# AIBluefisher/DAGSfM

Measured on AMD Instinct MI355X. Metric: verified image-pairs/sec (+ RANSAC hypotheses/sec) at 4096 feats/image, higher is better.
Workload: dtype u8 matching (int8 MFMA) + f64 verification

## Files before the change

dagsfm_amd/capi.py:

```python
import ctypes
import os

import numpy as np

_HERE = os.path.dirname(os.path.abspath(__file__))
LIB_PATH = os.environ.get("DSM_LIB_PATH") or os.path.join(_HERE, "libdagsfm_mi355x.so")
CHECK_LIB_PATH = os.environ.get("DSM_CHECK_LIB_PATH") or os.path.join(_HERE, "libdagsfm_mi355x_check.so")

GATHER_LIB_PATH = os.path.join(_HERE, "libdagsfm_gather.so")

u8p = ctypes.POINTER(ctypes.c_uint8)
u32p = ctypes.POINTER(ctypes.c_uint32)
u64p = ctypes.POINTER(ctypes.c_uint64)
f32p = ctypes.POINTER(ctypes.c_float)


class DsmError(RuntimeError):
    pass


class MatchOptions(ctypes.Structure):
    _fields_ = [("max_ratio", ctypes.c_double), ("max_distance", ctypes.c_double),
                ("cross_check", ctypes.c_int32), ("max_num_matches", ctypes.c_int32)]

# ... 668 lines not shown
            "image_camera": np.array([cam_new[int(icam[i])] for i in images], np.uint32),
            "qvec": qvec[images].copy(), "tvec": tvec[images].copy(), "image_constant_pose": cpose, "image_constant_tvec": cmask,
            "point_ids": ids[points].copy(), "xyz": xyz[points].copy(), "point_constant": np.array(pconst, np.uint8),
            "track_offsets": np.concatenate([[0], np.cumsum([len(t) for t in tracks])]).astype(np.uint32),
            "obs_image": np.array([img_new[int(oimg[k])] for t in tracks for k in t], np.uint32),
            "obs_xy": (np.concatenate([oxy[t] for t in tracks]) if tracks else np.zeros((0, 2))).reshape(-1, 2),
            "image_index": np.array(images, np.int64), "camera_index": np.array(cams, np.int64),
            "point_index": np.array(points, np.int64)}


def absolute_pose_seed(problem, factor_index, user_seed=0):
    return int(lib().dsm_absolute_pose_seed(problem, factor_index, user_seed))


def absolute_pose_factors(options=None):
    o = options if options is not None else default_absolute_pose_options()
    n = int(lib().dsm_absolute_pose_factors(ctypes.byref(o), None, 0))
    out = np.zeros(max(n, 1))
    lib().dsm_absolute_pose_factors(ctypes.byref(o), out.ctypes.data, n)
    return out[:n].copy()


def absolute_pose_max_trials(options=None):
    o = options if options is not None else default_absolute_pose_options()
    return int(lib().dsm_absolute_pose_max_trials(ctypes.byref(o)))


def align_seed(i, j, direction, user_seed=0):
    return int(lib().dsm_align_seed(i, j, direction, user_seed))


PRODUCT_OPTION_KEYS = ("DSM_MATCH_CHUNK_ROWS", "DSM_VERIFY_CHUNK_PAIRS", "DSM_VERIFY_LANES", "DSM_VERIFY_INLINE_LO", "DSM_VERIFY_ITEM_MODE",
                       "DSM_LO_TAIL", "DSM_LO_TAIL_MODE", "DSM_VERIFY_GRID_DIV")
CHECK_OPTION_KEYS = ("DSM_K1_DOT4", "DSM_VERIFY_DEBUG", "DSM_SAMPLER_SERIAL", "DSM_LO_PREPARE_WAVE", "DSM_LO_JACOBI_GROUPS", "DSM_ROOTS_LDS",
                     "DSM_FINAL_WAVES", "DSM_VERIFY_LEGACY", "DSM_VERIFY_FIXED_BATCH", "DSM_VERIFY_LANE_SPLIT", "DSM_DEBUG_SAMPLER_MODE",
                     "DSM_VOCAB_ASSIGN_VALU", "DSM_VERIFY_HOST_LOOP", "DSM_SCORE_PREFILTER", "DSM_VERIFY_REPLAY_GRID", "DSM_REPLAY_LEGACY", "DSM_FLANN_GROUP", "DSM_FLANN_STATS", "DSM_ELU_LDS", "DSM_HYP_GRID", "DSM_SPEC_MARGIN",
                     "DSM_POSE_FULL")
DEBUG_OPTION_KEYS = PRODUCT_OPTION_KEYS


def check_requested():
    return os.environ.get("DSM_LIBRARY") == "check" or any(os.environ.get(k) is not None for k in CHECK_OPTION_KEYS)


class Context:

    def __init__(self, device=0, check=None):
        self._handle = ctypes.c_void_p()
        self._debug = {}
        self.check = check_requested() if check is None else bool(check)
        self._L = lib(self.check)
        rc = self._L.dsm_ctx_create(device, ctypes.byref(self._handle))
        if rc != 0:
            raise DsmError("dsm_ctx_create failed (%d): %s" % (rc, self._L.dsm_last_error(None).decode()))
        self.n_pairs = 0

    @property
    def _h(self):
        if self._handle:
            for key in PRODUCT_OPTION_KEYS + CHECK_OPTION_KEYS:
                want = os.environ.get(key)
                if self._debug.get(key) != want:
                    self.set_debug_option(key, want)
        return self._handle

    def set_memory_budget(self, nbytes):
        self._L.dsm_ctx_set_memory_budget.argtypes = [ctypes.c_void_p, ctypes.c_uint64]
# ... 858 lines not shown
```

dagsfm_amd/csrc/capi.hip:

```cpp
#include <hip/hip_runtime.h>
#include <math.h>
#include <stdint.h>
#include <stdio.h>
#include <stdlib.h>
#include <string.h>

#include <algorithm>
#include <string>
#include <system_error>
#include <thread>
#include <vector>

#include "../../include/dagsfm_mi355x.h"
#include "ctx.h"
#include "kernels.h"
#include "verify_camera.h"

namespace {
thread_local std::string g_create_error;
}

static const uint64_t kStageSlot = 16ull << 20;
static const uint64_t kStageSmall = 1ull << 20;
static const unsigned kStageThreads = 8;
// ... 428 lines not shown
    uint32_t c1 = c0;
    while (c1 < n_pairs) {
      const uint64_t r = ctx->rows[pairs[2 * c1]];
      if (c1 > c0 && rows_acc + r > budget_rows) break;
      rows_acc += r;
      ++c1;
    }
    const uint32_t nc = c1 - c0;
    dpairs.resize(nc);
    dpairs2.resize(nc);
    pdir.resize(nc);
    doff.resize(nc);
    order.resize(nc);
    std::fill(cnt_b.begin(), cnt_b.end(), 0u);
    uint64_t off = 0;
    uint32_t max_rb = 0;
    for (uint32_t k = 0; k < nc; ++k) {
      const uint32_t a = pairs[2 * (c0 + k)], b = pairs[2 * (c0 + k) + 1];
      dpairs[k] = make_uint2(a, b);
      dpairs2[k] = make_uint2(b, a);
      pdir[k] = make_uint4(k, 0, ctx->nfeat[a], ctx->nfeat[b]);
      doff[k] = off;
      off += ctx->rows[a];
      max_rb = std::max(max_rb, ctx->rows[a] / 256);
      cnt_b[b + 1]++;
    }
    for (uint32_t k = 0; k < ctx->n_images; ++k) cnt_b[k + 1] += cnt_b[k];
    for (uint32_t k = 0; k < nc; ++k) order[cnt_b[dpairs[k].y]++] = k;
    HIPCHK(ctx, ctx->d_dpairs.reserve(std::max<uint32_t>(nc, 1) * sizeof(uint2)));
    HIPCHK(ctx, ctx->d_order.reserve(std::max<uint32_t>(nc, 1) * 4));
    HIPCHK(ctx, ctx->d_doutoff.reserve(std::max<uint32_t>(nc, 1) * 8));
    HIPCHK(ctx, ctx->d_pair_dir.reserve(std::max<uint32_t>(nc, 1) * sizeof(uint4)));
    HIPCHK(ctx, ctx->d_m.reserve(std::max<uint64_t>(off, 1) * 4));
    HIPCHK(ctx, ctx->d_ms.reserve(std::max<uint64_t>(off, 1) * 4));
    HIPCHK(ctx, hipMemcpyAsync(ctx->d_dpairs.p, dpairs.data(), nc * sizeof(uint2), hipMemcpyHostToDevice, st));
    HIPCHK(ctx, hipMemcpyAsync(ctx->d_order.p, order.data(), nc * 4, hipMemcpyHostToDevice, st));
    HIPCHK(ctx, hipMemcpyAsync(ctx->d_doutoff.p, doff.data(), nc * 8, hipMemcpyHostToDevice, st));
    HIPCHK(ctx, hipMemcpyAsync(ctx->d_pair_dir.p, pdir.data(), nc * sizeof(uint4), hipMemcpyHostToDevice, st));

    K1Params k1;
    k1.desc = ctx->d_desc.as<int8_t>();
    k1.rterm = ctx->d_rterm.as<int32_t>();
    k1.dpairs = ctx->d_dpairs.as<uint2>();
    k1.img_row0 = ctx->d_img_row0.as<uint32_t>();
    k1.img_rows = ctx->d_img_rows.as<uint32_t>();
    k1.d_out_off = ctx->d_doutoff.as<uint64_t>();
    k1.lut = ctx->d_lut.as<float>();
    k1.max_ratio = (float)options->max_ratio;
    k1.max_distance = (float)options->max_distance;
    k1.out = ctx->d_m.as<int32_t>();
    k1.out_s = ctx->d_ms.as<int32_t>();
    k1.order = ctx->d_order.as<uint32_t>();
    k1.entries = nullptr;
    k1.e_off = nullptr;
    k1.e_cnt = nullptr;
    while (ctx->ev.size() < ev_used + 6) {
      DevEvent e;
      HIPCHK(ctx, hipEventCreate(&e.e));
      ctx->ev.push_back(std::move(e));
    }
#ifdef DSM_CHECK_BUILD
    const bool k1_dot4 = ctx->dbg("DSM_K1_DOT4") != nullptr;
#else
    const bool k1_dot4 = false;
#endif
    HIPCHK(ctx, hipEventRecord(ctx->ev[ev_used], st));
#ifdef DSM_CHECK_BUILD
    if (k1_dot4)
      launch_k1_dot4(k1, nc, max_rb, st);
    else
#endif
      launch_k1(k1, nc, max_rb, st);
    HIPCHK(ctx, hipGetLastError());
    HIPCHK(ctx, hipEventRecord(ctx->ev[ev_used + 1], st));
    if (!k1_dot4) launch_k1_resolve(k1, nc, max_rb, st);
    HIPCHK(ctx, hipGetLastError());
    HIPCHK(ctx, hipEventRecord(ctx->ev[ev_used + 2], st));
    if (max_rb) ctx->k1_launches++;

    K2Params k2;
    k2.pair_dir = ctx->d_pair_dir.as<uint4>();
    k2.d_out_off = ctx->d_doutoff.as<uint64_t>();
    k2.m = ctx->d_m.as<int32_t>();
    k2.cross_check = 0;
    k2.matches = nullptr;
    uint64_t total = 0;
    if (!cross) {
      HIPCHK(ctx, hipEventRecord(ctx->ev[ev_used + 3], st));
      HIPCHK(ctx, hipEventRecord(ctx->ev[ev_used + 4], st));
      k2.counts = ctx->d_counts.as<uint32_t>() + c0;
      k2.offsets = ctx->d_offsets.as<uint64_t>() + c0;
      launch_k2(k2, nc, false, st);
      HIPCHK(ctx, hipGetLastError());
      launch_scan(ctx->d_counts.as<uint32_t>() + c0, ctx->d_offsets.as<uint64_t>() + c0, nc, ctx->d_total.as<uint64_t>(), st);
      HIPCHK(ctx, hipGetLastError());
      HIPCHK(ctx, hipMemcpyAsync(&total, ctx->d_total.p, 8, hipMemcpyDeviceToHost, st));
      HIPCHK(ctx, hipStreamSynchronize(st));
      HIPCHK(ctx, ctx->d_matches.grow(std::max<uint64_t>(total, 1) * 8, ctx->total_matches * 8, st));
      k2.matches = ctx->d_matches.as<uint32_t>();
      launch_k2(k2, nc, true, st);
      HIPCHK(ctx, hipGetLastError());
    } else {
      HIPCHK(ctx, ctx->d_ecnt.reserve(std::max<uint32_t>(nc, 1) * 4));
      HIPCHK(ctx, ctx->d_eoff.reserve(((size_t)nc + 1) * 8));
      HIPCHK(ctx, ctx->d_etotal.reserve(8));
      HIPCHK(ctx, hipMemsetAsync(ctx->d_etotal.p, 0, 8, st));
      k2.counts = ctx->d_ecnt.as<uint32_t>();
      k2.offsets = ctx->d_eoff.as<uint64_t>();
      launch_k2(k2, nc, false, st);
      HIPCHK(ctx, hipGetLastError());
      launch_scan(ctx->d_ecnt.as<uint32_t>(), ctx->d_eoff.as<uint64_t>(), nc, ctx->d_etotal.as<uint64_t>(), st);
      HIPCHK(ctx, hipGetLastError());
      uint64_t etotal = 0;
      HIPCHK(ctx, hipMemcpyAsync(&etotal, ctx->d_etotal.p, 8, hipMemcpyDeviceToHost, st));
      HIPCHK(ctx, hipStreamSynchronize(st));
      HIPCHK(ctx, ctx->d_entries.reserve(std::max<uint64_t>(etotal, 1) * 8));
      HIPCHK(ctx, ctx->d_out2.reserve(std::max<uint64_t>(etotal, 1) * 4));
      HIPCHK(ctx, ctx->d_out2s.reserve(std::max<uint64_t>(etotal, 1) * 4));
      k2.matches = ctx->d_entries.as<uint32_t>();
      launch_k2(k2, nc, true, st);
      HIPCHK(ctx, hipGetLastError());
      HIPCHK(ctx, ctx->d_dpairs2.reserve(std::max<uint32_t>(nc, 1) * sizeof(uint2)));
      HIPCHK(ctx, hipMemcpyAsync(ctx->d_dpairs2.p, dpairs2.data(), nc * sizeof(uint2), hipMemcpyHostToDevice, st));
      K1Params g = k1;
      g.dpairs = ctx->d_dpairs2.as<uint2>();
      g.order = nullptr;
      g.entries = ctx->d_entries.as<uint2>();
      g.e_off = ctx->d_eoff.as<uint64_t>();
      g.e_cnt = ctx->d_ecnt.as<uint32_t>();
      g.out = ctx->d_out2.as<int32_t>();
      g.out_s = ctx->d_out2s.as<int32_t>();
      HIPCHK(ctx, hipEventRecord(ctx->ev[ev_used + 3], st));
      if (etotal) {
        launch_k1(g, nc, max_rb, st);
        HIPCHK(ctx, hipGetLastError());
      }
      HIPCHK(ctx, hipEventRecord(ctx->ev[ev_used + 4], st));
      if (etotal) {
        launch_k1_resolve(g, nc, max_rb, st);
        HIPCHK(ctx, hipGetLastError());
      }
      K2eParams ke;
      ke.entries = g.entries;
      ke.e_off = g.e_off;
      ke.e_cnt = g.e_cnt;
      ke.out2 = ctx->d_out2.as<int32_t>();
      ke.counts = ctx->d_counts.as<uint32_t>() + c0;
      ke.offsets = ctx->d_offsets.as<uint64_t>() + c0;
      ke.matches = nullptr;
      launch_k2_entries(ke, nc, false, st);
      HIPCHK(ctx, hipGetLastError());
      launch_scan(ctx->d_counts.as<uint32_t>() + c0, ctx->d_offsets.as<uint64_t>() + c0, nc, ctx->d_total.as<uint64_t>(), st);
      HIPCHK(ctx, hipGetLastError());
      HIPCHK(ctx, hipMemcpyAsync(&total, ctx->d_total.p, 8, hipMemcpyDeviceToHost, st));
      HIPCHK(ctx, hipStreamSynchronize(st));
      HIPCHK(ctx, ctx->d_matches.grow(std::max<uint64_t>(total, 1) * 8, ctx->total_matches * 8, st));
      ke.matches = ctx->d_matches.as<uint32_t>();
      launch_k2_entries(ke, nc, true, st);
      HIPCHK(ctx, hipGetLastError());
    }
    HIPCHK(ctx, hipEventRecord(ctx->ev[ev_used + 5], st));
    ev_used += 6;
    ctx->total_matches = total;
    HIPCHK(ctx, hipStreamSynchronize(st));
    c0 = c1;
  }
  HIPCHK(ctx, hipStreamSynchronize(st));
  for (size_t k = 0; k + 5 < ev_used; k += 6) {
    float ms = 0.f;
    HIPCHK(ctx, hipEventElapsedTime(&ms, ctx->ev[k + 4], ctx->ev[k + 5]));
    ctx->k1t_ms += ms;
    HIPCHK(ctx, hipEventElapsedTime(&ms, ctx->ev[k + 2], ctx->ev[k + 3]));
    ctx->k1t_ms += ms;
    HIPCHK(ctx, hipEventElapsedTime(&ms, ctx->ev[k], ctx->ev[k + 1]));
// ... 1243 lines not shown
```

dagsfm_amd/csrc/ctx.h:

```cpp
#ifndef DAGSFM_AMD_CSRC_CTX_H_
#define DAGSFM_AMD_CSRC_CTX_H_

#include <hip/hip_runtime.h>
#include <stdint.h>

#include <map>
#include <string>
#include <vector>

#include "../../include/dagsfm_mi355x.h"

struct DevBuf {
  void* p = nullptr;
  size_t cap = 0;
  DevBuf() = default;
  DevBuf(const DevBuf&) = delete;
  DevBuf& operator=(const DevBuf&) = delete;
  DevBuf(DevBuf&& o) noexcept : p(o.p), cap(o.cap) {
    o.p = nullptr;
    o.cap = 0;
  }
  DevBuf& operator=(DevBuf&& o) noexcept {
    if (this != &o) {
      release();
// ... 167 lines not shown

  struct RetrievalState* retrieval = nullptr;
  struct CovSiftState* covsift = nullptr;
  struct SiftState* sift = nullptr;

  std::vector<double> cluster_ritz, cluster_vectors;
  uint32_t cluster_rows = 0, cluster_cols = 0;

  template <typename F>
  void for_each_buffer(F f) {
    for (DevBuf* b : {&d_desc, &d_rterm, &d_kp, &d_img_row0, &d_img_rows, &d_lut, &d_stage, &d_counts, &d_offsets, &d_matches, &d_total, &d_etotal,
                      &d_cams, &d_pairs_dev, &d_seeds, &d_tvg, &d_inl, &d_inl_counts, &d_inl_off, &d_inl_compact, &d_inl_total, &d_nt_table,
                      &d_nt_off, &d_nt_off_t, &d_pair_state, &d_pts_px, &d_pts_norm, &d_reports, &d_masks, &d_fam_state, &d_sidx, &d_lo_inl,
                      &d_nt_table_t, &d_wm_redo, &d_wm_total, &d_wm_count, &d_lo_inl_pool, &d_pose_jobs,
                      &d_g_nfeat, &d_g_dpairs, &d_g_doff, &d_g_pdir, &d_g_params, &d_g_m, &d_g_counts, &d_g_offsets, &d_g_total, &d_g_matches,
                      &d_g_plan, &d_g_inl, &d_g_inl_off,
                      &d_mm_matches[0], &d_mm_matches[1], &d_mm_off[0], &d_mm_off[1], &d_mm_counts, &d_mm_state, &d_mm_first, &d_mm_acc,
                      &d_mm_keep, &d_mm_total})
      f(*b, false);
    for (DevBuf* b : {&d_m, &d_ms, &d_entries, &d_out2, &d_out2s, &d_dpairs, &d_dpairs2, &d_doutoff, &d_pair_dir, &d_order, &d_ecnt, &d_eoff,
                      &d_vscratch})
      f(*b, true);
    for (VerifyLane& L : lanes) L.for_each_buffer([&f](DevBuf& b) { f(b, true); });
  }
};
void dsm_retrieval_destroy(dsm_ctx* ctx);
void dsm_retrieval_invalidate(dsm_ctx* ctx);
void dsm_sift_destroy(dsm_ctx* ctx);
void dsm_covariant_sift_destroy(dsm_ctx* ctx);

static const char* const dsm_product_debug_keys[] = {"DSM_MATCH_CHUNK_ROWS", "DSM_VERIFY_CHUNK_PAIRS", "DSM_VERIFY_LANES", "DSM_VERIFY_INLINE_LO",
                                                     "DSM_VERIFY_ITEM_MODE", "DSM_LO_TAIL", "DSM_LO_TAIL_MODE", "DSM_VERIFY_GRID_DIV"};
#ifdef DSM_CHECK_BUILD
static const char* const dsm_check_debug_keys[] = {"DSM_K1_DOT4", "DSM_VERIFY_DEBUG", "DSM_SAMPLER_SERIAL", "DSM_LO_PREPARE_WAVE", "DSM_LO_JACOBI_GROUPS",
                                                   "DSM_ROOTS_LDS", "DSM_FINAL_WAVES", "DSM_VERIFY_LEGACY", "DSM_VERIFY_FIXED_BATCH", "DSM_VERIFY_LANE_SPLIT",
                                                   "DSM_DEBUG_SAMPLER_MODE", "DSM_VOCAB_ASSIGN_VALU", "DSM_VERIFY_HOST_LOOP", "DSM_SCORE_PREFILTER",
                                                   "DSM_VERIFY_REPLAY_GRID", "DSM_REPLAY_LEGACY", "DSM_FLANN_GROUP", "DSM_FLANN_STATS", "DSM_ELU_LDS", "DSM_HYP_GRID", "DSM_SPEC_MARGIN",
                                                   "DSM_POSE_FULL"};
#endif

#define HIPCHK(ctx, call)                                                              \
  do {                                                                                 \
    hipError_t e_ = (call);                                                            \
    if (e_ != hipSuccess) {                                                            \
      (ctx)->err = std::string(#call) + ": " + hipGetErrorString(e_);                  \
      return DSM_ERR_HIP;                                                              \
    }                                                                                  \
  } while (0)

#define HIPTRY(call)                                                   \
  do {                                                                 \
    hipError_t e_ = (call);                                            \
    if (e_ != hipSuccess && rc == DSM_OK) {                            \
      ctx->err = std::string(#call) + ": " + hipGetErrorString(e_);    \
      rc = DSM_ERR_HIP;                                                \
    }                                                                  \
  } while (0)

static inline int dsm_fail(dsm_ctx* ctx, int code, const char* msg) {
  if (ctx) ctx->err = msg;
  return code;
}

#endif
```

dagsfm_amd/csrc/kernels.h:

```cpp
#ifndef DAGSFM_AMD_CSRC_KERNELS_H_
#define DAGSFM_AMD_CSRC_KERNELS_H_

#include <hip/hip_runtime.h>
#include <stdint.h>

#include "../../include/dagsfm_mi355x.h"

struct K1Params {
  const int8_t* desc;
  const int32_t* rterm;
  const uint2* dpairs;
  const uint32_t* img_row0;
  const uint32_t* img_rows;
  const uint64_t* d_out_off;
  const float* lut;
  float max_ratio;
  float max_distance;
  int32_t* out;
  int32_t* out_s;
  const uint32_t* order;
  const uint2* entries;
  const uint64_t* e_off;
  const uint32_t* e_cnt;
};
// ... 160 lines not shown
  uint32_t* lo_count;
  double* lo_work;
  double* lo_models;
  double* lo_slots;
  double* lo_ework;
};

size_t verify_scratch_bytes_per_block(uint32_t n_max);
size_t verify_smem_bytes(uint32_t n_max);
void launch_verify(const VerifyParams& p, uint32_t n_blocks, hipStream_t st);
void launch_vp_prep(const VerifyParams& p, uint32_t n_blocks, hipStream_t st);
void launch_vp_sample(const VerifyParams& p, int fam, uint32_t n_blocks, hipStream_t st);
void launch_vp_solve_score(const VerifyParams& p, int fam, hipStream_t st);
void launch_vp_replay(const VerifyParams& p, int fam, uint32_t n_blocks, hipStream_t st);
void launch_vp_final(const VerifyParams& p, uint32_t n_blocks, hipStream_t st);
void launch_vp_replay_lo(const VerifyParams& p, int fam, uint32_t n_blocks, int mode, hipStream_t st);
void launch_vp_items_enum(const VerifyParams& p, int fam, hipStream_t st);
void launch_vp_items_inliers(const VerifyParams& p, int fam, uint32_t n_blocks, hipStream_t st);
void launch_vp_items_outcome(const VerifyParams& p, int fam, uint32_t n_blocks, hipStream_t st);
void launch_vp_local_opt(const VerifyParams& p, int fam, uint32_t n_blocks, uint32_t n_wave_prepare, uint32_t n_small_jacobi, uint32_t n_big_prepare, hipStream_t st);
void launch_lane_counters(const void* src, uint32_t* dst_host, uint32_t copy_bytes, void* zero, size_t zero_bytes, hipStream_t st);
uint32_t vp_batch(int fam, uint32_t max_trials, uint32_t min_trials);
uint32_t vp_maxm(int fam);
void debug_read_prof(unsigned long long* out16);
void launch_debug_samples(uint32_t seed, uint32_t k, uint32_t total, uint32_t n_draws, uint32_t* out, uint32_t* idx, uint32_t* tmp7,
                          int mode, hipStream_t st);
void launch_debug_image_to_world(const dsm_camera& cam, uint32_t n, const double* xy, double* uv, hipStream_t st);
void launch_compact_inliers(const uint64_t* match_off, const uint64_t* inl_off, const uint32_t* inl_counts,
                            const uint32_t* src, uint32_t* dst, uint32_t n_pairs, hipStream_t st);

void launch_k0(const uint8_t* in_u8, int8_t* out_s8, int32_t* rterm, uint64_t n_rows, hipStream_t st);
void launch_k1(const K1Params& p, uint32_t n_directed, uint32_t max_row_blocks, hipStream_t st);
void launch_k1_dot4(const K1Params& p, uint32_t n_directed, uint32_t max_row_blocks, hipStream_t st);
void launch_k1_resolve(const K1Params& p, uint32_t n_directed, uint32_t max_row_blocks, hipStream_t st);
void launch_k2(const K2Params& p, uint32_t n_pairs, bool write, hipStream_t st);
void launch_k2_entries(const K2eParams& p, uint32_t n_pairs, bool write, hipStream_t st);
void launch_scan(const uint32_t* counts, uint64_t* offsets, uint32_t n, uint64_t* running_total, hipStream_t st);

struct MultiState {
  uint32_t ngeo;
  uint32_t done;
  uint32_t acc_inl;
  uint32_t pad;
  uint32_t trials[4], models[4];
};
struct MultiParams {
  const uint64_t* cur_off;
  const uint32_t* cur_matches;
  const uint64_t* orig_off;
  const dsm_two_view_geometry* tvg;
  const uint32_t* inl;
  const uint32_t* inl_counts;
  MultiState* state;
  dsm_two_view_geometry* first;
  uint32_t* acc;
  unsigned char* keep;
  uint32_t* next_count;
  const uint64_t* next_off;
  uint32_t* next_matches;
  uint32_t* active;
  int32_t ignore_watermark;
  int32_t stage_filter;
  uint64_t min_num_inliers;
  uint32_t n_pairs;
  dsm_two_view_geometry* out_tvg;
  uint32_t* out_inl_counts;
// ... 7 lines not shown
```

dagsfm_amd/csrc/match_kernels.hip:

```cpp
#include <hip/hip_runtime.h>
#include <stdint.h>

#include <type_traits>

#include "kernels.h"

typedef int v4i __attribute__((ext_vector_type(4)));
typedef int v16i __attribute__((ext_vector_type(16)));

template <int B, int E, typename F>
__device__ __forceinline__ void static_for(F&& f) {
  if constexpr (B < E) {
    f(std::integral_constant<int, B>());
    static_for<B + 1, E>(f);
  }
}

__global__ __launch_bounds__(256) void k0_prepare(const uint8_t* __restrict__ in_u8,
                                                  int8_t* __restrict__ out_s8,
                                                  int32_t* __restrict__ rterm,
                                                  uint64_t n_rows) {
  const uint64_t gid = (uint64_t)blockIdx.x * blockDim.x + threadIdx.x;
  const uint64_t row = gid >> 3;
  const uint32_t chunk = (uint32_t)gid & 7u;
// ... 26 lines not shown
        : [a0] "v"(a[0]), [a1] "v"(a[1]), [a2] "v"(a[2]), [a3] "v"(a[3]), [a4] "v"(a[4]), [a5] "v"(a[5]), [a6] "v"(a[6]));
  } else if constexpr (Q == 1) {
    asm volatile(
        "v_max3_i32 %[t], %[t], %[a0], %[a1]\n\t"
        "v_max3_i32 %[t], %[t], %[a2], %[a3]\n\t"
        "v_max3_i32 %[t], %[t], %[a4], %[a5]"
        : [t] "+v"(t)
        : [a0] "v"(a[7]), [a1] "v"(a[8]), [a2] "v"(a[9]), [a3] "v"(a[10]), [a4] "v"(a[11]), [a5] "v"(a[12]));
  } else if constexpr (Q == 2) {
    asm volatile(
        "v_max3_i32 %[t], %[t], %[a0], %[a1]\n\t"
        "v_max3_i32 %[t], %[t], %[a2], %[s]\n\t"
        "v_min_i32 %[s], %[t], %[b]"
        : [t] "+v"(t), [s] "+v"(second)
        : [b] "v"(best), [a0] "v"(a[13]), [a1] "v"(a[14]), [a2] "v"(a[15]));
  } else {
    asm volatile(
        "v_cmp_gt_i32 vcc, %[t], %[b]\n\t"
        "v_cndmask_b32 %[bt], %[bt], %[tile], vcc\n\t"
        "v_max_i32 %[b], %[t], %[b]"
        : [b] "+v"(best), [bt] "+v"(btile)
        : [t] "v"(t), [tile] "v"(tile)
        : "vcc");
  }
}

#ifndef K1_LDS_DMA
#define K1_LDS_DMA 0
#endif
__device__ __forceinline__ int lds_off(int col, int chunk) {
  return col * 128 + ((chunk ^ ((col >> 1) & 7)) << 4);
}

template <bool GATHER>
__global__ __launch_bounds__(256, 2) void k1_best_rows(const K1Params p) {
  const uint32_t d = p.order ? p.order[blockIdx.x] : blockIdx.x;
  const uint32_t rb = blockIdx.y;
  const uint2 ab = p.dpairs[d];
  const uint32_t a_rows = GATHER ? p.e_cnt[d] : p.img_rows[ab.x];
  if (rb * 512u >= a_rows) return;
  const uint32_t b_cols = p.img_rows[ab.y];
  const uint32_t a_row0 = (GATHER ? 0u : p.img_row0[ab.x]) + rb * 512u;
  const uint32_t b_row0 = p.img_row0[ab.y];

  const int tid = threadIdx.x;
  const int lane = tid & 63;
  const int wave = tid >> 6;
  const int l31 = lane & 31;
  const int half = lane >> 5;
  const bool active = rb * 512u + (uint32_t)wave * 128u < a_rows;

  __shared__ __attribute__((aligned(16))) int8_t sB[2][64 * 128];
  __shared__ __attribute__((aligned(16))) int sC[2][64];

  v4i afrag[4][4];
  int rterm_i[4];
  bool valid[4];
  {
    const uint2* ent = GATHER ? p.entries + p.e_off[d] : nullptr;
    const uint32_t img0 = GATHER ? p.img_row0[ab.x] : 0u;
#pragma unroll
    for (int rt = 0; rt < 4; ++rt) {
      const uint32_t r = a_row0 + wave * 128 + rt * 32 + l31;
      valid[rt] = GATHER ? (r < a_rows) : active;
      uint32_t grow = r;
      if (GATHER) grow = valid[rt] ? img0 + ent[r].y : 0u;
      const int8_t* arow = p.desc + (size_t)grow * 128;
// ... 97 lines not shown
      static_for<0, 4>([&](auto KS) { K1_MFMA(0, KS.value); });
      __builtin_amdgcn_sched_barrier(0);
      static_for<0, 28>([&](auto J) {
        constexpr int j = J.value;
        K1_MFMA((j >> 2) + 1, j & 3);
        __builtin_amdgcn_sched_barrier(0);
        if constexpr (j >= 1) {
          K1_EPI(j - 1);
          __builtin_amdgcn_sched_barrier(0);
        }
      });
      static_for<27, 32>([&](auto E) { K1_EPI(E.value); });
      __builtin_amdgcn_sched_barrier(0);
#undef K1_MFMA
#undef K1_EPI
    }
    if (more) {
#if !K1_LDS_DMA
#pragma unroll
      for (int u = 0; u < 2; ++u) {
        const int q = tid + 256 * u;
        *reinterpret_cast<v4i*>(&sB[cur ^ 1][lds_off(q >> 3, q & 7)]) = stage[u];
      }
#endif
      if (tid < 64) sC[cur ^ 1][tid] = cstage + (1 << 21);
    }
    __syncthreads();
  }

  if (!active) return;
  const uint64_t out0 = (GATHER ? p.e_off[d] : p.d_out_off[d]) + rb * 512u + wave * 128;
  int32_t* out = p.out + out0;
  int32_t* out_s = p.out_s + out0;
#pragma unroll
  for (int rt = 0; rt < 4; ++rt) {
    const int oB = __shfl_xor(best[rt], 32);
    const int oS = __shfl_xor(second[rt], 32);
    const int oT = __shfl_xor(btile[rt], 32);
    const int B = max(best[rt], oB);
    const int S = max(min(best[rt], oB), max(second[rt], oS));
    const bool take = (oB > best[rt]) || (oB == best[rt] && oT < btile[rt]);
    const bool both = oB == best[rt] && oT == btile[rt];
    const int T = take ? oT : btile[rt];
    const int set = both ? 2 : ((take ? 1 : 0) ^ half);
    const int best_dot = B + rterm_i[rt];
    const int second_dot = S + rterm_i[rt];
    int res = -1;
    if (best_dot > 0) {
      const float bn = p.lut[min(best_dot, 262144)];
      if (!(bn > p.max_distance)) {
        const float sn = p.lut[min(second_dot, 262144)];
        const float rhs = __fmul_rn(p.max_ratio, sn);
        if (!(bn >= rhs)) res = T * 4 + set;
      }
    }
    if (half == (rt & 1) && valid[rt]) {
      out[rt * 32 + l31] = res;
      if (res >= 0) out_s[rt * 32 + l31] = second_dot;
    }
  }
}

template <bool GATHER>
__global__ __launch_bounds__(256) void k1_resolve_index(const K1Params p) {
  const uint32_t d = blockIdx.x;
  const uint2 ab = p.dpairs[d];
  const uint32_t a_rows = GATHER ? p.e_cnt[d] : p.img_rows[ab.x];
  const int tid = threadIdx.x;
  const int lane = tid & 63, wave = tid >> 6;
  const uint32_t b_row0 = p.img_row0[ab.y];
  const uint32_t a_img0 = p.img_row0[ab.x];
  const int8_t* bimg = p.desc + (size_t)b_row0 * 128;
  const int32_t* rt_b = p.rterm + b_row0;
  const uint2* ent = GATHER ? p.entries + p.e_off[d] : nullptr;
  const int g = lane >> 3;
  for (uint32_t row_w = wave * 64u; row_w < a_rows; row_w += 256u) {
    const uint64_t o0 = (GATHER ? p.e_off[d] : p.d_out_off[d]) + row_w;
    int32_t* out = p.out + o0;
    const int32_t* out_s = p.out_s + o0;
    const bool in_range = !GATHER || row_w + (uint32_t)lane < a_rows;
    const int t = in_range ? out[lane] : -1;
    const int s_appr = t >= 0 ? out_s[lane] : 0;
    const uint32_t my_row = GATHER ? (in_range ? ent[row_w + lane].y : 0u) : row_w + (uint32_t)lane;
    unsigned long long mask = __ballot(t >= 0);
    constexpr int RU = 4;
    while (mask) {
      int r_l[RU], tile_l[RU], set_l[RU], sap_l[RU];
      uint32_t grow_l[RU];
      bool on[RU];
#pragma unroll
      for (int u = 0; u < RU; ++u) {
        on[u] = mask != 0ull;
        const int r = on[u] ? (__ffsll((long long)mask) - 1) : 0;
        if (on[u]) mask &= mask - 1;
        r_l[u] = r;
        const int code = on[u] ? __builtin_amdgcn_readlane(t, r) : 0;
        tile_l[u] = code >> 2;
        set_l[u] = code & 3;
        sap_l[u] = __builtin_amdgcn_readlane(s_appr, r);
        grow_l[u] = a_img0 + (uint32_t)__builtin_amdgcn_readlane((int)my_row, r);
      }
      v4i x[RU], y[RU][4];
      int ct[RU][4], col[RU][4], rti[RU];
#pragma unroll
      for (int u = 0; u < RU; ++u) {
        x[u] = *reinterpret_cast<const v4i*>(p.desc + (size_t)grow_l[u] * 128 + (lane & 7) * 16);
        rti[u] = p.rterm[grow_l[u]];
        const bool both = set_l[u] == 2;
#pragma unroll
        for (int i = 0; i < 4; ++i) {
          col[u][i] = both ? i * 8 + g : 8 * (2 * (i & 1) + (g >> 2)) + 4 * set_l[u] + (g & 3);
          if (i < 2 || both) {
            const int c = tile_l[u] * 32 + col[u][i];
            y[u][i] = *reinterpret_cast<const v4i*>(bimg + (size_t)c * 128 + (lane & 7) * 16);
            ct[u][i] = rt_b[c];
          }
        }
      }
#pragma unroll
      for (int u = 0; u < RU; ++u) {
        const bool both = set_l[u] == 2;
        int k1 = INT32_MIN, k2 = INT32_MIN;
#pragma unroll
        for (int i = 0; i < 4; ++i) {
          if (i < 2 || both) {
            int acc = 0;
#pragma unroll
            for (int e = 0; e < 4; ++e) acc = __builtin_amdgcn_sdot4(x[u][e], y[u][i][e], acc, false);
            acc += __shfl_xor(acc, 1);
            acc += __shfl_xor(acc, 2);
            acc += __shfl_xor(acc, 4);
            const int key = (int)((uint32_t)(acc + ct[u][i]) << 5) | (31 - col[u][i]);
            k2 = max(k2, min(k1, key));
            k1 = max(k1, key);
          }
        }
#pragma unroll
        for (int o = 8; o < 64; o <<= 1) {
          const int o1 = __shfl_xor(k1, o), o2 = __shfl_xor(k2, o);
          k2 = max(min(k1, o1), max(k2, o2));
          k1 = max(k1, o1);
        }
        if (lane == 0 && on[u]) {
          const int bias = rti[u] + (1 << 21);
          const int best_dot = (k1 >> 5) + bias;
          const int second_dot = max(sap_l[u], (k2 >> 5) + bias);
          const float bn = p.lut[min(best_dot, 262144)];
          const float sn = p.lut[min(second_dot, 262144)];
          const float rhs = __fmul_rn(p.max_ratio, sn);
          out[r_l[u]] = (bn >= rhs) ? -1 : tile_l[u] * 32 + (31 - (k1 & 31));
        }
      }
    }
  }
}

#ifdef DSM_CHECK_BUILD
__global__ __launch_bounds__(256) void k1_best_rows_dot4(const K1Params p) {
  const uint32_t d = p.order ? p.order[blockIdx.x] : blockIdx.x;
  const uint32_t rb = blockIdx.y;
  const uint2 ab = p.dpairs[d];
  const uint32_t a_rows = p.img_rows[ab.x];
  if (rb * 512u >= a_rows) return;
  const uint32_t b_cols = p.img_rows[ab.y];
  const uint32_t a_row0 = p.img_row0[ab.x], b_row0 = p.img_row0[ab.y];
  const int tid = threadIdx.x;
  const uint32_t row[2] = {rb * 512u + tid, rb * 512u + 256u + tid};
  const bool has2 = row[1] < a_rows;
  __shared__ __attribute__((aligned(16))) int8_t sB[2][64 * 128];
  __shared__ int sR[2][64];
  v4i a[2][8];
  int rterm_i[2];
#pragma unroll
  for (int r = 0; r < 2; ++r) {
    const uint32_t rr = (r == 0 || has2) ? row[r] : row[0];
    const int8_t* arow = p.desc + (size_t)(a_row0 + rr) * 128;
#pragma unroll
    for (int c = 0; c < 8; ++c) a[r][c] = *reinterpret_cast<const v4i*>(arow + c * 16);
    rterm_i[r] = p.rterm[a_row0 + rr];
  }
  int best[2] = {0, 0}, second[2] = {0, 0}, best_j[2] = {-1, -1};
  const uint32_t nsteps = b_cols >> 6;
  v4i st[2];
  int sr = 0;
  auto fetch = [&](uint32_t s) {
// ... 254 lines not shown
    for (int o = 1; o < 64; o <<= 1) {
      const uint64_t y = __shfl_up(x, o);
      if (lane >= o) x += y;
    }
    if (lane == 63) wsum[wave] = x;
    __syncthreads();
    uint64_t wbase = 0, total = 0;
#pragma unroll
    for (int w = 0; w < 16; ++w) {
      if (w < wave) wbase += wsum[w];
      total += wsum[w];
    }
    if (i < n) offsets[i] = carry + wbase + x - v;
    __syncthreads();
    if (tid == 0) carry += total;
    __syncthreads();
  }
  if (tid == 0) {
    offsets[n] = carry;
    *running_total = carry;
  }
}

void launch_k0(const uint8_t* in_u8, int8_t* out_s8, int32_t* rterm, uint64_t n_rows, hipStream_t st) {
  if (n_rows == 0) return;
  const uint64_t threads = n_rows * 8;
  const uint32_t blocks = (uint32_t)((threads + 255) / 256);
  hipLaunchKernelGGL(k0_prepare, dim3(blocks), dim3(256), 0, st, in_u8, out_s8, rterm, n_rows);
}

void launch_k1(const K1Params& p, uint32_t n_directed, uint32_t max_row_blocks, hipStream_t st) {
  if (n_directed == 0 || max_row_blocks == 0) return;
  if (p.entries)
    hipLaunchKernelGGL(k1_best_rows<true>, dim3(n_directed, (max_row_blocks + 1) / 2), dim3(256), 0, st, p);
  else
    hipLaunchKernelGGL(k1_best_rows<false>, dim3(n_directed, (max_row_blocks + 1) / 2), dim3(256), 0, st, p);
}
#ifdef DSM_CHECK_BUILD
void launch_k1_dot4(const K1Params& p, uint32_t n_directed, uint32_t max_row_blocks, hipStream_t st) {
  if (n_directed == 0 || max_row_blocks == 0) return;
  hipLaunchKernelGGL(k1_best_rows_dot4, dim3(n_directed, (max_row_blocks + 1) / 2), dim3(256), 0, st, p);
}
#endif
void launch_k1_resolve(const K1Params& p, uint32_t n_directed, uint32_t max_row_blocks, hipStream_t st) {
  if (n_directed == 0 || max_row_blocks == 0) return;
  if (p.entries)
    hipLaunchKernelGGL(k1_resolve_index<true>, dim3(n_directed), dim3(256), 0, st, p);
  else
    hipLaunchKernelGGL(k1_resolve_index<false>, dim3(n_directed), dim3(256), 0, st, p);
}
void launch_k2_entries(const K2eParams& p, uint32_t n_pairs, bool write, hipStream_t st) {
  if (n_pairs == 0) return;
  if (write)
    hipLaunchKernelGGL(k2_entries_compact<true>, dim3(n_pairs), dim3(256), 0, st, p);
  else
    hipLaunchKernelGGL(k2_entries_compact<false>, dim3(n_pairs), dim3(256), 0, st, p);
}

void launch_kg(const KgParams& p, uint32_t n_directed, uint32_t max_row_blocks, hipStream_t st) {
  if (n_directed == 0 || max_row_blocks == 0) return;
  hipLaunchKernelGGL(kg_best_rows, dim3(n_directed, max_row_blocks), dim3(256), 0, st, p);
}

struct GuidedPlan {
  uint64_t src_off, dst_off;
  uint32_t count, from_guided;
};
__global__ __launch_bounds__(64) void k_guided_assemble(const GuidedPlan* plan, const uint32_t* old_inl, const uint32_t* guided,
                                                        uint32_t* dst, uint32_t n_pairs) {
  for (uint32_t pi = blockIdx.x; pi < n_pairs; pi += gridDim.x) {
    const GuidedPlan pl = plan[pi];
    const uint2* s = reinterpret_cast<const uint2*>(pl.from_guided ? guided : old_inl) + pl.src_off;
    uint2* d = reinterpret_cast<uint2*>(dst) + pl.dst_off;
    for (uint32_t i = threadIdx.x; i < pl.count; i += 64) d[i] = s[i];
  }
}
void launch_guided_assemble(const void* plan, const uint32_t* old_inl, const uint32_t* guided, uint32_t* dst, uint32_t n_pairs,
                            hipStream_t st) {
  if (!n_pairs) return;
  hipLaunchKernelGGL(k_guided_assemble, dim3(n_pairs < 8192 ? n_pairs : 8192), dim3(64), 0, st,
                     static_cast<const GuidedPlan*>(plan), old_inl, guided, dst, n_pairs);
}

// ... 12 lines not shown
```

Before: 271,700.

## Fuse k1 best-row resolve into the MFMA match kernel via LDS-staged A rows

```diff
diff --git a/dagsfm_amd/capi.py b/dagsfm_amd/capi.py
--- a/dagsfm_amd/capi.py
+++ b/dagsfm_amd/capi.py
@@ -724,7 +724,7 @@
 
 PRODUCT_OPTION_KEYS = ("DSM_MATCH_CHUNK_ROWS", "DSM_VERIFY_CHUNK_PAIRS", "DSM_VERIFY_LANES", "DSM_VERIFY_INLINE_LO", "DSM_VERIFY_ITEM_MODE",
                        "DSM_LO_TAIL", "DSM_LO_TAIL_MODE", "DSM_VERIFY_GRID_DIV")
-CHECK_OPTION_KEYS = ("DSM_K1_DOT4", "DSM_VERIFY_DEBUG", "DSM_SAMPLER_SERIAL", "DSM_LO_PREPARE_WAVE", "DSM_LO_JACOBI_GROUPS", "DSM_ROOTS_LDS",
+CHECK_OPTION_KEYS = ("DSM_K1_DOT4", "DSM_K1_RESOLVE_KERNEL", "DSM_VERIFY_DEBUG", "DSM_SAMPLER_SERIAL", "DSM_LO_PREPARE_WAVE", "DSM_LO_JACOBI_GROUPS", "DSM_ROOTS_LDS",
                      "DSM_FINAL_WAVES", "DSM_VERIFY_LEGACY", "DSM_VERIFY_FIXED_BATCH", "DSM_VERIFY_LANE_SPLIT", "DSM_DEBUG_SAMPLER_MODE",
                      "DSM_VOCAB_ASSIGN_VALU", "DSM_VERIFY_HOST_LOOP", "DSM_SCORE_PREFILTER", "DSM_VERIFY_REPLAY_GRID", "DSM_REPLAY_LEGACY", "DSM_FLANN_GROUP", "DSM_FLANN_STATS", "DSM_ELU_LDS", "DSM_HYP_GRID", "DSM_SPEC_MARGIN",
                      "DSM_POSE_FULL")
diff --git a/dagsfm_amd/csrc/capi.hip b/dagsfm_amd/csrc/capi.hip
--- a/dagsfm_amd/csrc/capi.hip
+++ b/dagsfm_amd/csrc/capi.hip
@@ -484,7 +484,6 @@
     HIPCHK(ctx, ctx->d_doutoff.reserve(std::max<uint32_t>(nc, 1) * 8));
     HIPCHK(ctx, ctx->d_pair_dir.reserve(std::max<uint32_t>(nc, 1) * sizeof(uint4)));
     HIPCHK(ctx, ctx->d_m.reserve(std::max<uint64_t>(off, 1) * 4));
-    HIPCHK(ctx, ctx->d_ms.reserve(std::max<uint64_t>(off, 1) * 4));
     HIPCHK(ctx, hipMemcpyAsync(ctx->d_dpairs.p, dpairs.data(), nc * sizeof(uint2), hipMemcpyHostToDevice, st));
     HIPCHK(ctx, hipMemcpyAsync(ctx->d_order.p, order.data(), nc * 4, hipMemcpyHostToDevice, st));
     HIPCHK(ctx, hipMemcpyAsync(ctx->d_doutoff.p, doff.data(), nc * 8, hipMemcpyHostToDevice, st));
@@ -501,7 +500,7 @@
     k1.max_ratio = (float)options->max_ratio;
     k1.max_distance = (float)options->max_distance;
     k1.out = ctx->d_m.as<int32_t>();
-    k1.out_s = ctx->d_ms.as<int32_t>();
+    k1.out_s = nullptr;
     k1.order = ctx->d_order.as<uint32_t>();
     k1.entries = nullptr;
     k1.e_off = nullptr;
@@ -513,20 +512,27 @@
     }
 #ifdef DSM_CHECK_BUILD
     const bool k1_dot4 = ctx->dbg("DSM_K1_DOT4") != nullptr;
-#else
-    const bool k1_dot4 = false;
+    const bool k1_two = ctx->dbg("DSM_K1_RESOLVE_KERNEL") != nullptr;
+    if (k1_two) {
+      HIPCHK(ctx, ctx->d_ms.reserve(std::max<uint64_t>(off, 1) * 4));
+      k1.out_s = ctx->d_ms.as<int32_t>();
+    }
 #endif
     HIPCHK(ctx, hipEventRecord(ctx->ev[ev_used], st));
 #ifdef DSM_CHECK_BUILD
     if (k1_dot4)
       launch_k1_dot4(k1, nc, max_rb, st);
+    else if (k1_two)
+      launch_k1_unfused(k1, nc, max_rb, st);
     else
 #endif
       launch_k1(k1, nc, max_rb, st);
     HIPCHK(ctx, hipGetLastError());
     HIPCHK(ctx, hipEventRecord(ctx->ev[ev_used + 1], st));
-    if (!k1_dot4) launch_k1_resolve(k1, nc, max_rb, st);
+#ifdef DSM_CHECK_BUILD
+    if (k1_two && !k1_dot4) launch_k1_resolve(k1, nc, max_rb, st);
     HIPCHK(ctx, hipGetLastError());
+#endif
     HIPCHK(ctx, hipEventRecord(ctx->ev[ev_used + 2], st));
     if (max_rb) ctx->k1_launches++;
 
@@ -568,7 +574,6 @@
       HIPCHK(ctx, hipStreamSynchronize(st));
       HIPCHK(ctx, ctx->d_entries.reserve(std::max<uint64_t>(etotal, 1) * 8));
       HIPCHK(ctx, ctx->d_out2.reserve(std::max<uint64_t>(etotal, 1) * 4));
-      HIPCHK(ctx, ctx->d_out2s.reserve(std::max<uint64_t>(etotal, 1) * 4));
       k2.matches = ctx->d_entries.as<uint32_t>();
       launch_k2(k2, nc, true, st);
       HIPCHK(ctx, hipGetLastError());
@@ -581,17 +586,29 @@
       g.e_off = ctx->d_eoff.as<uint64_t>();
       g.e_cnt = ctx->d_ecnt.as<uint32_t>();
       g.out = ctx->d_out2.as<int32_t>();
-      g.out_s = ctx->d_out2s.as<int32_t>();
+#ifdef DSM_CHECK_BUILD
+      if (k1_two) {
+        HIPCHK(ctx, ctx->d_out2s.reserve(std::max<uint64_t>(etotal, 1) * 4));
+        g.out_s = ctx->d_out2s.as<int32_t>();
+      }
+#endif
       HIPCHK(ctx, hipEventRecord(ctx->ev[ev_used + 3], st));
       if (etotal) {
-        launch_k1(g, nc, max_rb, st);
+#ifdef DSM_CHECK_BUILD
+        if (k1_two)
+          launch_k1_unfused(g, nc, max_rb, st);
+        else
+#endif
+          launch_k1(g, nc, max_rb, st);
         HIPCHK(ctx, hipGetLastError());
       }
       HIPCHK(ctx, hipEventRecord(ctx->ev[ev_used + 4], st));
-      if (etotal) {
+#ifdef DSM_CHECK_BUILD
+      if (etotal && k1_two) {
         launch_k1_resolve(g, nc, max_rb, st);
         HIPCHK(ctx, hipGetLastError());
       }
+#endif
       K2eParams ke;
       ke.entries = g.entries;
       ke.e_off = g.e_off;
diff --git a/dagsfm_amd/csrc/ctx.h b/dagsfm_amd/csrc/ctx.h
--- a/dagsfm_amd/csrc/ctx.h
+++ b/dagsfm_amd/csrc/ctx.h
@@ -223,7 +223,7 @@
 static const char* const dsm_product_debug_keys[] = {"DSM_MATCH_CHUNK_ROWS", "DSM_VERIFY_CHUNK_PAIRS", "DSM_VERIFY_LANES", "DSM_VERIFY_INLINE_LO",
                                                      "DSM_VERIFY_ITEM_MODE", "DSM_LO_TAIL", "DSM_LO_TAIL_MODE", "DSM_VERIFY_GRID_DIV"};
 #ifdef DSM_CHECK_BUILD
-static const char* const dsm_check_debug_keys[] = {"DSM_K1_DOT4", "DSM_VERIFY_DEBUG", "DSM_SAMPLER_SERIAL", "DSM_LO_PREPARE_WAVE", "DSM_LO_JACOBI_GROUPS",
+static const char* const dsm_check_debug_keys[] = {"DSM_K1_DOT4", "DSM_K1_RESOLVE_KERNEL", "DSM_VERIFY_DEBUG", "DSM_SAMPLER_SERIAL", "DSM_LO_PREPARE_WAVE", "DSM_LO_JACOBI_GROUPS",
                                                    "DSM_ROOTS_LDS", "DSM_FINAL_WAVES", "DSM_VERIFY_LEGACY", "DSM_VERIFY_FIXED_BATCH", "DSM_VERIFY_LANE_SPLIT",
                                                    "DSM_DEBUG_SAMPLER_MODE", "DSM_VOCAB_ASSIGN_VALU", "DSM_VERIFY_HOST_LOOP", "DSM_SCORE_PREFILTER",
                                                    "DSM_VERIFY_REPLAY_GRID", "DSM_REPLAY_LEGACY", "DSM_FLANN_GROUP", "DSM_FLANN_STATS", "DSM_ELU_LDS", "DSM_HYP_GRID", "DSM_SPEC_MARGIN",
diff --git a/dagsfm_amd/csrc/kernels.h b/dagsfm_amd/csrc/kernels.h
--- a/dagsfm_amd/csrc/kernels.h
+++ b/dagsfm_amd/csrc/kernels.h
@@ -216,6 +216,7 @@
 void launch_k0(const uint8_t* in_u8, int8_t* out_s8, int32_t* rterm, uint64_t n_rows, hipStream_t st);
 void launch_k1(const K1Params& p, uint32_t n_directed, uint32_t max_row_blocks, hipStream_t st);
 void launch_k1_dot4(const K1Params& p, uint32_t n_directed, uint32_t max_row_blocks, hipStream_t st);
+void launch_k1_unfused(const K1Params& p, uint32_t n_directed, uint32_t max_row_blocks, hipStream_t st);
 void launch_k1_resolve(const K1Params& p, uint32_t n_directed, uint32_t max_row_blocks, hipStream_t st);
 void launch_k2(const K2Params& p, uint32_t n_pairs, bool write, hipStream_t st);
 void launch_k2_entries(const K2eParams& p, uint32_t n_pairs, bool write, hipStream_t st);
diff --git a/dagsfm_amd/csrc/match_kernels.hip b/dagsfm_amd/csrc/match_kernels.hip
--- a/dagsfm_amd/csrc/match_kernels.hip
+++ b/dagsfm_amd/csrc/match_kernels.hip
@@ -82,7 +82,82 @@
   return col * 128 + ((chunk ^ ((col >> 1) & 7)) << 4);
 }
 
-template <bool GATHER>
+template <int CTRL>
+__device__ __forceinline__ int k1_dpp(int v) {
+  return __builtin_amdgcn_update_dpp(0, v, CTRL, 0xf, 0xf, false);
+}
+template <int RU, bool BOTH, typename LoadRow>
+__device__ __forceinline__ void k1_resolve_keys(const int8_t* bimg, const int32_t* rt_b, int lane, int n, const int (&tile_l)[RU],
+                                                const int (&set_l)[RU], LoadRow&& load_row, int (&k1_l)[RU], int (&k2_l)[RU]) {
+  constexpr int XOR1 = 0xB1, XOR2 = 0x4E, HALF_MIRROR = 0x141, MIRROR = 0x140;
+  const int g = lane >> 3;
+  constexpr int NL = BOTH ? 4 : 2;
+  v4i x[RU], y[RU][NL];
+  int ct[RU][NL], col[RU][NL];
+#pragma unroll
+  for (int u = 0; u < RU; ++u) {
+    if (u >= n) break;
+    x[u] = load_row(u);
+    const bool both = BOTH && set_l[u] == 2;
+#pragma unroll
+    for (int i = 0; i < NL; ++i) {
+      col[u][i] = both ? i * 8 + g : 8 * (2 * (i & 1) + (g >> 2)) + 4 * set_l[u] + (g & 3);
+      if (i < 2 || both) {
+        const int c = tile_l[u] * 32 + col[u][i];
+        y[u][i] = *reinterpret_cast<const v4i*>(bimg + (size_t)c * 128 + (lane & 7) * 16);
+        ct[u][i] = rt_b[c];
+      }
+    }
+  }
+#pragma unroll
+  for (int u = 0; u < RU; ++u) {
+    if (u >= n) break;
+    const bool both = BOTH && set_l[u] == 2;
+    int k1 = INT32_MIN, k2 = INT32_MIN;
+#pragma unroll
+    for (int i = 0; i < NL; ++i) {
+      if (i < 2 || both) {
+        int acc = 0;
+#pragma unroll
+        for (int e = 0; e < 4; ++e) acc = __builtin_amdgcn_sdot4(x[u][e], y[u][i][e], acc, false);
+        acc += k1_dpp<XOR1>(acc);
+        acc += k1_dpp<XOR2>(acc);
+        acc += k1_dpp<HALF_MIRROR>(acc);
+        const int key = (int)((uint32_t)(acc + ct[u][i]) << 5) | (31 - col[u][i]);
+        k2 = max(k2, min(k1, key));
+        k1 = max(k1, key);
+      }
+    }
+    {
+      const int o1 = k1_dpp<MIRROR>(k1), o2 = k1_dpp<MIRROR>(k2);
+      k2 = max(min(k1, o1), max(k2, o2));
+      k1 = max(k1, o1);
+    }
+    int s1 = __builtin_amdgcn_readlane(k1, 0), s2 = __builtin_amdgcn_readlane(k2, 0);
+#pragma unroll
+    for (int o = 16; o < 64; o += 16) {
+      const int o1 = __builtin_amdgcn_readlane(k1, o), o2 = __builtin_amdgcn_readlane(k2, o);
+      s2 = max(min(s1, o1), max(s2, o2));
+      s1 = max(s1, o1);
+    }
+    k1_l[u] = s1;
+    k2_l[u] = s2;
+  }
+}
+__device__ __forceinline__ int k1_resolve_final(const K1Params& p, int k1, int k2, int sap, int rti, int tile) {
+  const int bias = rti + (1 << 21);
+  const int best_dot = (k1 >> 5) + bias;
+  const int second_dot = max(sap, (k2 >> 5) + bias);
+  const float bn = p.lut[min(best_dot, 262144)];
+  const float sn = p.lut[min(second_dot, 262144)];
+  const float rhs = __fmul_rn(p.max_ratio, sn);
+  return (bn >= rhs) ? -1 : tile * 32 + (31 - (k1 & 31));
+}
+
+#ifndef K1_TAIL_RU
+#define K1_TAIL_RU 6
+#endif
+template <bool GATHER, bool FUSED>
 __global__ __launch_bounds__(256, 2) void k1_best_rows(const K1Params p) {
   const uint32_t d = p.order ? p.order[blockIdx.x] : blockIdx.x;
   const uint32_t rb = blockIdx.y;
@@ -246,6 +321,7 @@
   const uint64_t out0 = (GATHER ? p.e_off[d] : p.d_out_off[d]) + rb * 512u + wave * 128;
   int32_t* out = p.out + out0;
   int32_t* out_s = p.out_s + out0;
+  int res_f[4], sdot_f[4];
 #pragma unroll
   for (int rt = 0; rt < 4; ++rt) {
     const int oB = __shfl_xor(best[rt], 32);
@@ -268,9 +344,81 @@
         if (!(bn >= rhs)) res = T * 4 + set;
       }
     }
-    if (half == (rt & 1) && valid[rt]) {
-      out[rt * 32 + l31] = res;
-      if (res >= 0) out_s[rt * 32 + l31] = second_dot;
+    if constexpr (!FUSED) {
+      if (half == (rt & 1) && valid[rt]) {
+        out[rt * 32 + l31] = res;
+        if (res >= 0) out_s[rt * 32 + l31] = second_dot;
+      }
+    } else {
+      res_f[rt] = res;
+      sdot_f[rt] = second_dot;
+    }
+  }
+  if constexpr (FUSED) {
+    int lane_t = lane;
+    asm volatile("" : "+v"(lane_t));
+    const int l31_t = lane_t & 31, half_t = lane_t >> 5;
+    int8_t* slice = &sB[0][0] + wave * 4096;
+    int k1v[4] = {0, 0, 0, 0}, k2v[4] = {0, 0, 0, 0};
+#pragma nounroll
+    for (int rt = 0; rt < 4; ++rt) {
+      int res = -1, k1c = 0, k2c = 0;
+      static_for<0, 4>([&](auto RT) {
+        if (rt == RT.value) res = res_f[RT.value];
+      });
+      const uint32_t mask = (uint32_t)__ballot(res >= 0);
+      if (mask == 0u) continue;
+      __builtin_amdgcn_fence(__ATOMIC_RELEASE, "wavefront");
+      static_for<0, 4>([&](auto RT) {
+        if (rt == RT.value) {
+#pragma unroll
+          for (int ks = 0; ks < 4; ++ks)
+            *reinterpret_cast<v4i*>(slice + l31_t * 128 + (((ks * 2 + half_t) ^ (l31_t & 7)) << 4)) = afrag[RT.value][ks];
+        }
+      });
+      __builtin_amdgcn_fence(__ATOMIC_ACQ_REL, "wavefront");
+      uint32_t mask_b = (uint32_t)__ballot(res >= 0 && (res & 3) == 2);
+      uint32_t mask_n = mask & ~mask_b;
+      auto trips = [&](auto RU_, auto BOTH_, uint32_t m) {
+        constexpr int RU = decltype(RU_)::value;
+        while (m) {
+          int r_l[RU], tile_l[RU], set_l[RU], k1_l[RU], k2_l[RU];
+          bool on[RU];
+          const int n = min(__popc(m), RU);
+#pragma unroll
+          for (int u = 0; u < RU; ++u) {
+            on[u] = m != 0u;
+            const int r = on[u] ? (__ffs((int)m) - 1) : 0;
+            if (on[u]) m &= m - 1;
+            r_l[u] = r;
+            const int code = on[u] ? __builtin_amdgcn_readlane(res, r) : 0;
+            tile_l[u] = code >> 2;
+            set_l[u] = code & 3;
+          }
+          k1_resolve_keys<RU, decltype(BOTH_)::value>(
+              bimg, rt_b, lane_t, n, tile_l, set_l,
+              [&](int u) { return *reinterpret_cast<const v4i*>(slice + r_l[u] * 128 + (((lane_t & 7) ^ (r_l[u] & 7)) << 4)); }, k1_l, k2_l);
+#pragma unroll
+          for (int u = 0; u < RU; ++u)
+            if (on[u] && l31_t == r_l[u]) {
+              k1c = k1_l[u];
+              k2c = k2_l[u];
+            }
+        }
+      };
+      trips(std::integral_constant<int, K1_TAIL_RU>(), std::false_type(), mask_n);
+      trips(std::integral_constant<int, 4>(), std::true_type(), mask_b);
+      static_for<0, 4>([&](auto RT) {
+        if (rt == RT.value) {
+          k1v[RT.value] = k1c;
+          k2v[RT.value] = k2c;
+        }
+      });
+    }
+#pragma unroll
+    for (int rt = 0; rt < 4; ++rt) {
+      const int col = k1_resolve_final(p, k1v[rt], k2v[rt], sdot_f[rt], rterm_i[rt], res_f[rt] >> 2);
+      if (half_t == (rt & 1) && valid[rt]) out[rt * 32 + l31_t] = res_f[rt] >= 0 ? col : -1;
     }
   }
 }
@@ -287,7 +435,6 @@
   const int8_t* bimg = p.desc + (size_t)b_row0 * 128;
   const int32_t* rt_b = p.rterm + b_row0;
   const uint2* ent = GATHER ? p.entries + p.e_off[d] : nullptr;
-  const int g = lane >> 3;
   for (uint32_t row_w = wave * 64u; row_w < a_rows; row_w += 256u) {
     const uint64_t o0 = (GATHER ? p.e_off[d] : p.d_out_off[d]) + row_w;
     int32_t* out = p.out + o0;
@@ -299,9 +446,10 @@
     unsigned long long mask = __ballot(t >= 0);
     constexpr int RU = 4;
     while (mask) {
-      int r_l[RU], tile_l[RU], set_l[RU], sap_l[RU];
+      int r_l[RU], tile_l[RU], set_l[RU], sap_l[RU], rti_l[RU], k1_l[RU], k2_l[RU];
       uint32_t grow_l[RU];
       bool on[RU];
+      const int n = min(__popcll(mask), RU);
 #pragma unroll
       for (int u = 0; u < RU; ++u) {
         on[u] = mask != 0ull;
@@ -313,58 +461,14 @@
         set_l[u] = code & 3;
         sap_l[u] = __builtin_amdgcn_readlane(s_appr, r);
         grow_l[u] = a_img0 + (uint32_t)__builtin_amdgcn_readlane((int)my_row, r);
-      }
-      v4i x[RU], y[RU][4];
-      int ct[RU][4], col[RU][4], rti[RU];
-#pragma unroll
-      for (int u = 0; u < RU; ++u) {
-        x[u] = *reinterpret_cast<const v4i*>(p.desc + (size_t)grow_l[u] * 128 + (lane & 7) * 16);
-        rti[u] = p.rterm[grow_l[u]];
-        const bool both = set_l[u] == 2;
-#pragma unroll
-        for (int i = 0; i < 4; ++i) {
-          col[u][i] = both ? i * 8 + g : 8 * (2 * (i & 1) + (g >> 2)) + 4 * set_l[u] + (g & 3);
-          if (i < 2 || both) {
-            const int c = tile_l[u] * 32 + col[u][i];
-            y[u][i] = *reinterpret_cast<const v4i*>(bimg + (size_t)c * 128 + (lane & 7) * 16);
-            ct[u][i] = rt_b[c];
-          }
-        }
-      }
-#pragma unroll
-      for (int u = 0; u < RU; ++u) {
-        const bool both = set_l[u] == 2;
-        int k1 = INT32_MIN, k2 = INT32_MIN;
-#pragma unroll
-        for (int i = 0; i < 4; ++i) {
-          if (i < 2 || both) {
-            int acc = 0;
-#pragma unroll
-            for (int e = 0; e < 4; ++e) acc = __builtin_amdgcn_sdot4(x[u][e], y[u][i][e], acc, false);
-            acc += __shfl_xor(acc, 1);
-            acc += __shfl_xor(acc, 2);
-            acc += __shfl_xor(acc, 4);
-            const int key = (int)((uint32_t)(acc + ct[u][i]) << 5) | (31 - col[u][i]);
-            k2 = max(k2, min(k1, key));
-            k1 = max(k1, key);
-          }
-        }
-#pragma unroll
-        for (int o = 8; o < 64; o <<= 1) {
-          const int o1 = __shfl_xor(k1, o), o2 = __shfl_xor(k2, o);
-          k2 = max(min(k1, o1), max(k2, o2));
-          k1 = max(k1, o1);
-        }
-        if (lane == 0 && on[u]) {
-          const int bias = rti[u] + (1 << 21);
-          const int best_dot = (k1 >> 5) + bias;
-          const int second_dot = max(sap_l[u], (k2 >> 5) + bias);
-          const float bn = p.lut[min(best_dot, 262144)];
-          const float sn = p.lut[min(second_dot, 262144)];
-          const float rhs = __fmul_rn(p.max_ratio, sn);
-          out[r_l[u]] = (bn >= rhs) ? -1 : tile_l[u] * 32 + (31 - (k1 & 31));
-        }
-      }
+        rti_l[u] = p.rterm[grow_l[u]];
+      }
+      k1_resolve_keys<RU, true>(bimg, rt_b, lane, n, tile_l, set_l,
+                                [&](int u) { return *reinterpret_cast<const v4i*>(p.desc + (size_t)grow_l[u] * 128 + (lane & 7) * 16); },
+                                k1_l, k2_l);
+#pragma unroll
+      for (int u = 0; u < RU; ++u)
+        if (lane == 0 && on[u]) out[r_l[u]] = k1_resolve_final(p, k1_l[u], k2_l[u], sap_l[u], rti_l[u], tile_l[u]);
     }
   }
 }
@@ -685,16 +789,18 @@
 void launch_k1(const K1Params& p, uint32_t n_directed, uint32_t max_row_blocks, hipStream_t st) {
   if (n_directed == 0 || max_row_blocks == 0) return;
   if (p.entries)
-    hipLaunchKernelGGL(k1_best_rows<true>, dim3(n_directed, (max_row_blocks + 1) / 2), dim3(256), 0, st, p);
+    hipLaunchKernelGGL((k1_best_rows<true, true>), dim3(n_directed, (max_row_blocks + 1) / 2), dim3(256), 0, st, p);
   else
-    hipLaunchKernelGGL(k1_best_rows<false>, dim3(n_directed, (max_row_blocks + 1) / 2), dim3(256), 0, st, p);
+    hipLaunchKernelGGL((k1_best_rows<false, true>), dim3(n_directed, (max_row_blocks + 1) / 2), dim3(256), 0, st, p);
 }
 #ifdef DSM_CHECK_BUILD
-void launch_k1_dot4(const K1Params& p, uint32_t n_directed, uint32_t max_row_blocks, hipStream_t st) {
+void launch_k1_unfused(const K1Params& p, uint32_t n_directed, uint32_t max_row_blocks, hipStream_t st) {
   if (n_directed == 0 || max_row_blocks == 0) return;
-  hipLaunchKernelGGL(k1_best_rows_dot4, dim3(n_directed, (max_row_blocks + 1) / 2), dim3(256), 0, st, p);
-}
-#endif
+  if (p.entries)
+    hipLaunchKernelGGL((k1_best_rows<true, false>), dim3(n_directed, (max_row_blocks + 1) / 2), dim3(256), 0, st, p);
+  else
+    hipLaunchKernelGGL((k1_best_rows<false, false>), dim3(n_directed, (max_row_blocks + 1) / 2), dim3(256), 0, st, p);
+}
 void launch_k1_resolve(const K1Params& p, uint32_t n_directed, uint32_t max_row_blocks, hipStream_t st) {
   if (n_directed == 0 || max_row_blocks == 0) return;
   if (p.entries)
@@ -702,6 +808,11 @@
   else
     hipLaunchKernelGGL(k1_resolve_index<false>, dim3(n_directed), dim3(256), 0, st, p);
 }
+void launch_k1_dot4(const K1Params& p, uint32_t n_directed, uint32_t max_row_blocks, hipStream_t st) {
+  if (n_directed == 0 || max_row_blocks == 0) return;
+  hipLaunchKernelGGL(k1_best_rows_dot4, dim3(n_directed, (max_row_blocks + 1) / 2), dim3(256), 0, st, p);
+}
+#endif
 void launch_k2_entries(const K2eParams& p, uint32_t n_pairs, bool write, hipStream_t st) {
   if (n_pairs == 0) return;
   if (write)
```

New measurement: 279,100 (median of 6 runs). 2.7% higher.
